# RainbowZL0/swin-unet-image-fusion

Hardware: AMD Instinct MI355X
Metric: fused image-pairs/sec at 256x256, win=8 (higher is better)
Workload: dtype bf16; 1 GPU; B=16/GPU 256x256 IR/visible pairs, win=8, 5-level Swin-UNet fusion forward (BASELINE configs[1]); global_batch=16, precision_mode=fast, residual_stream=fp32, hip_graph=True, steps_in_flight=3, kernel_schedule=throughput, collective=none, weights=random-init (numpy PCG64 recipe, seed 0)

## Files before the change

### swin_unet_image_fusion_amd/csrc/kernels_win24.hip

```cpp
#include "win_host.h"

namespace swf {
namespace {

using namespace wf;

constexpr int W24_WAVES = 3;

template <int HID_>
struct G24 {
    static constexpr int C = 24, HID = HID_, HEADS = 8, D = 3;
    static constexpr bool ONES_H = HID % 32 != 0;
    static constexpr int NT1 = (HID + (ONES_H ? 1 : 0) + 31) / 32;
    static constexpr int KU = (HID + (ONES_H ? 1 : 0) + 15) / 16;
    static constexpr int F_QKV = 0;
    static constexpr int F_P = 12;
    static constexpr int F_W1 = 16;
    static constexpr int F_W2 = F_W1 + 4 * NT1;
    static constexpr int NFRAG = F_W2 + 2 * KU;
    static constexpr size_t p_vec = size_t(NFRAG) * 1024;
    static constexpr int V_LN1G = 0, V_LN1B = 12, V_LN2G = 24, V_LN2B = 36, V_B2 = 48;
    static constexpr size_t p_bias = p_vec + 2 * 64 * 4;
    static constexpr size_t p_total = p_bias + size_t(2) * 2 * 16 * 64 * 4;
    static constexpr size_t l_k = 0, l_v = l_k + 16 * 1024, l_vec = l_v + 16 * 1024, l_total = l_vec + 2 * 2 * 64 * 4;
    static constexpr size_t p_total16 = p_bias + size_t(15) * 64 * 16 * 4;
    static constexpr size_t l_k16 = 0, l_v16 = 32 * 1024, l_vec16 = 64 * 1024, l_total16 = l_vec16 + 2 * 2 * 64 * 4;
};

__device__ __forceinline__ void layernorm_frags(const f32x16& res, const float* vec, int goff, int boff, u32x4 (&xh)[2], u32x4 (&xl)[2]) {
    float s = 0.f;
#pragma unroll
    for (int i = 0; i < 12; ++i) s += res[i];
    const float mean = sum_halves(s) * (1.0f / 24.0f);
    float d[12], q = 0.f;
#pragma unroll
    for (int i = 0; i < 12; ++i) {
        d[i] = res[i] - mean;
        q += d[i] * d[i];
    }
    const float rstd = __builtin_amdgcn_rsqf(sum_halves(q) * (1.0f / 24.0f) + 1e-5f);
    float n[16];
#pragma unroll
    for (int a = 0; a < 3; ++a) {
        const float4 g = *reinterpret_cast<const float4*>(vec + goff + 4 * a);
        const float4 b = *reinterpret_cast<const float4*>(vec + boff + 4 * a);
        n[4 * a + 0] = d[4 * a + 0] * rstd * g.x + b.x;
        n[4 * a + 1] = d[4 * a + 1] * rstd * g.y + b.y;
        n[4 * a + 2] = d[4 * a + 2] * rstd * g.z + b.z;
        n[4 * a + 3] = d[4 * a + 3] * rstd * g.w + b.w;
    }
    n[12] = 1.0f;
    n[13] = n[14] = n[15] = 0.f;
    split8(n, xh[0], xl[0]);
    split8(n + 8, xh[1], xl[1]);
}

__device__ __forceinline__ void raw_frags(const f32x16& res, u32x4 (&xh)[2], u32x4 (&xl)[2]) {
    float n[16];
#pragma unroll
    for (int i = 0; i < 12; ++i) n[i] = res[i];
    n[12] = 1.0f;
    n[13] = n[14] = n[15] = 0.f;
    split8(n, xh[0], xl[0]);
    split8(n + 8, xh[1], xl[1]);
}

template <bool ONLINE>
__device__ __forceinline__ f32x16 attention24(const u32x4* ksrc, const u32x4* vsrc, const u32x4 (&qf)[2], const f32x16 (&bias)[2], bool half1,
                                            f32x16 o, float* mrun = nullptr) {
    const f32x16 zero16 = {0.f, 0.f, 0.f, 0.f, 0.f, 0.f, 0.f, 0.f, 0.f, 0.f, 0.f, 0.f, 0.f, 0.f, 0.f, 0.f};
#pragma unroll
    for (int h = 0; h < 8; ++h) {
        const int s = h >> 2, sub = (h >> 1) & 1;
        const bool keep = half1 == ((h & 1) != 0);
        const u32x4 ka0 = ksrc[(0 * 2 + s) * 64], ka1 = ksrc[(1 * 2 + s) * 64];
        u32x4 qm = {0u, 0u, 0u, 0u};
        qm[2 * sub] = keep ? qf[s][2 * sub] : 0u;
        qm[2 * sub + 1] = keep ? qf[s][2 * sub + 1] : 0u;
        f32x16 s0 = mfma_f16(ka0, qm, bias[0]);
        f32x16 s1 = mfma_f16(ka1, qm, bias[1]);
        float mx = max3f(s0[0], s0[1], s1[0]);
        mx = max3f(mx, s1[1], s0[2]);
#pragma unroll
        for (int i = 3; i < 16; i += 2) mx = max3f(mx, s0[i], s0[i + 1 < 16 ? i + 1 : i]);
#pragma unroll
        for (int i = 2; i < 16; i += 2) mx = max3f(mx, s1[i], s1[i + 1]);
        mx = max_halves(mx);
        float alpha = 0.f;
        f16 nm = (f16)(-mx);
        if constexpr (ONLINE) {
            const float mold = mrun[h >> 1];
            nm = (f16)(-__builtin_fmaxf(mold, mx));
            const float mnew = -(float)nm;
            alpha = __builtin_amdgcn_exp2f(mold - mnew);
            mrun[h >> 1] = keep ? mnew : mold;
        }
        const unsigned nmb = keep ? (unsigned)__builtin_bit_cast(unsigned short, nm) : 0u;
        qm[2 * sub + 1] |= nmb << 16;
        s0 = mfma_f16(ka0, qm, bias[0]);
        s1 = mfma_f16(ka1, qm, bias[1]);
        f32x16 t;
#pragma unroll
        for (int ps = 0; ps < 4; ++ps) {
            float p[8];
#pragma unroll
            for (int j = 0; j < 8; ++j) p[j] = __builtin_amdgcn_exp2f((ps >> 1) ? s1[8 * (ps & 1) + j] : s0[8 * (ps & 1) + j]);
            const u32x4 pf = pack8_f16(p);
            const u32x4 va = vsrc[ps * 64];
            t = mfma_f16(va, pf, ps == 0 ? zero16 : t);
            __builtin_amdgcn_sched_barrier(0);
        }
#pragma unroll
        for (int j = 0; j < 4; ++j) {
            const int i = 4 * (h >> 1) + j;
            o[i] = keep ? (ONLINE ? __builtin_fmaf(o[i], alpha, t[i]) : t[i]) : o[i];
        }
        __builtin_amdgcn_sched_barrier(0);
    }
    return o;
}

__device__ __forceinline__ void load_rows24(const __amdgpu_buffer_rsrc_t& irs, unsigned tokoff, f32x16& dstv) {
#pragma unroll
    for (int a = 0; a < 3; ++a) {
        const f32x4 v = __builtin_bit_cast(f32x4, __builtin_amdgcn_raw_buffer_load_b128(irs, tokoff, 32 * a, 0));
        dstv[4 * a] = v.x; dstv[4 * a + 1] = v.y; dstv[4 * a + 2] = v.z; dstv[4 * a + 3] = v.w;
    }
    dstv[12] = dstv[13] = dstv[14] = dstv[15] = 0.f;
}
__device__ __forceinline__ void store_rows24(__amdgpu_buffer_rsrc_t ors, unsigned tokoff, f32x16 res) {
#pragma unroll
    for (int a = 0; a < 3; ++a) {
        const f32x4 v = {res[4 * a], res[4 * a + 1], res[4 * a + 2], res[4 * a + 3]};
        __builtin_amdgcn_raw_buffer_store_b128(__builtin_bit_cast(u32x4, v), ors, tokoff, 32 * a, 0);
    }
}

template <class G, class WFn>
__device__ __forceinline__ f32x16 project24(WFn WF, f32x16 o, f32x16 res) {
    float t[16];
#pragma unroll
    for (int a = 0; a < 4; ++a) {
        const float inv = __builtin_amdgcn_rcpf(o[4 * a + 3]);
        t[4 * a] = o[4 * a] * inv; t[4 * a + 1] = o[4 * a + 1] * inv; t[4 * a + 2] = o[4 * a + 2] * inv;
        t[4 * a + 3] = 1.0f;
    }
    u32x4 oh[2], ol[2];
    split8(t, oh[0], ol[0]);
// ... 16 lines not shown
    u32x4* kimg = reinterpret_cast<u32x4*>(smem + G::l_k);
    u32x4* vimg = reinterpret_cast<u32x4*>(smem + G::l_v);
    float* lvec = reinterpret_cast<float*>(smem + G::l_vec);

    const int tid = threadIdx.x, lane = tid & 63, wave = tid >> 6;
    const int ws = wave >> 1, qb = wave & 1, r = lane & 31, hf = lane >> 5;
    const int H = args.H, W = args.W, nwx = MLP && !ATT ? 1 : W / WS, nwy = MLP && !ATT ? 1 : H / WS, npi = nwx * nwy;
    const int nwin = ATT ? args.B * npi : (max(args.ntok[0], args.ntok[1]) + 63) / 64;
    const int sh = args.shift ? WS / 2 : 0;
    const int kvs = args.cross ? 1 - ws : ws;

    for (int i = tid; i < 2 * 2 * 64; i += 256) lvec[i] = reinterpret_cast<const float*>(args.packed[i >> 7] + G::p_vec)[i & 127];
    const __amdgpu_buffer_rsrc_t wrs = __builtin_amdgcn_make_buffer_rsrc(const_cast<char*>(uniform_ptr(args.packed[ws])), 0, (int)G::p_total, 0x00020000);
    const __amdgpu_buffer_rsrc_t krs = __builtin_amdgcn_make_buffer_rsrc(const_cast<char*>(uniform_ptr(args.packed[kvs])), 0, (int)G::p_total, 0x00020000);
    const int act_bytes = ATT ? args.B * H * W * 24 * 4 : args.ntok[ws] * 24 * 4;
    const __amdgpu_buffer_rsrc_t irs = __builtin_amdgcn_make_buffer_rsrc(const_cast<float*>(uniform_ptr(args.in[ws])), 0, act_bytes, 0x00020000);
    const __amdgpu_buffer_rsrc_t ors = __builtin_amdgcn_make_buffer_rsrc(uniform_ptr(args.out[ws]), 0, (MODE == WIN_BLOCK || args.out[ws]) ? act_bytes : 0, 0x00020000);
    const unsigned loff = (unsigned)lane * 16u;
    auto WF = [&](int f) { return __builtin_bit_cast(u32x4, __builtin_amdgcn_raw_buffer_load_b128(wrs, loff, f * 1024, 0)); };
    auto WK = [&](int f) { return __builtin_bit_cast(u32x4, __builtin_amdgcn_raw_buffer_load_b128(krs, loff, f * 1024, 0)); };
    const float* vec = lvec + (ws * 2 + hf) * 64;
    f32x16 bias[2];
    auto load_bias = [&]() {
        const int vo = lane * 128 + qb * (2 * 16 * 64 * 4);
#pragma unroll
        for (int kt = 0; kt < 2; ++kt)
#pragma unroll
            for (int q4 = 0; q4 < 4; ++q4) {
                const f32x4 t = __builtin_bit_cast(f32x4, __builtin_amdgcn_raw_buffer_load_b128(wrs, vo + (kt * 16 + q4 * 4) * 4, (int)G::p_bias, 0));
#pragma unroll
                for (int e = 0; e < 4; ++e) bias[kt][q4 * 4 + e] = t[e];
            }
    };
    if constexpr (ATT) load_bias();
    const bool half1 = hf != 0;
    const bool col_masked = half1 != (((r >> 2) & 1) != 0);
    __syncthreads();

    int it = 0;
    for (int win = blockIdx.x; win < nwin; win += gridDim.x, ++it) {
        SWF_WF_FENCE();
        const int b = win / npi, wrem = win - b * npi;
        const int wy = wrem / nwx, wx = wrem - wy * nwx;
        const int buf = it & 1;
        int lane_w = lane;
        asm volatile("" : "+v"(lane_w));
        const int ty = 4 * qb + ((lane_w >> 3) & 3), tx = lane_w & 7;
        unsigned oy = wy * WS + ty + sh, ox = wx * WS + tx + sh;
        oy = oy < oy - (unsigned)H ? oy : oy - (unsigned)H;
        ox = ox < ox - (unsigned)W ? ox : ox - (unsigned)W;
        const unsigned tokoff = [&]() -> unsigned {
            if constexpr (ATT) {
                return (WS == 8 || (ty < WS && tx < WS)) ? (unsigned)((((b * H + (int)oy) * W + (int)ox) * 24 + 4 * (lane_w >> 5)) * 4) : 0x80000000u;
            } else {
                const int tok = 64 * win + 32 * qb + (lane_w & 31);
                return tok < args.ntok[ws] ? (unsigned)((tok * 24 + 4 * (lane_w >> 5)) * 4) : 0x80000000u;
            }
        }();
        const f32x16 zero16 = {0.f, 0.f, 0.f, 0.f, 0.f, 0.f, 0.f, 0.f, 0.f, 0.f, 0.f, 0.f, 0.f, 0.f, 0.f, 0.f};

        f32x16 res;
        if constexpr (ATT) {
        u32x4 qf[2];
        {
            f32x16 x0;
            load_rows24(irs, tokoff, x0);
            u32x4 xh[2], xl[2];
            if constexpr (RAW) raw_frags(x0, xh, xl);
            else layernorm_frags(x0, vec, G::V_LN1G, G::V_LN1B, xh, xl);
            f32x16 acc = zero16;
            if (!(RAW && ws == 1)) {
#pragma unroll
                for (int s = 0; s < 2; ++s) acc = mma3(WF(G::F_QKV + 2 * s), WF(G::F_QKV + 2 * s + 1), xh[s], xl[s], acc);
                float t[16];
#pragma unroll
                for (int i = 0; i < 16; ++i) t[i] = acc[i];
                qf[0] = pack8_f16(t);
                qf[1] = pack8_f16(t + 8);
            }
            SWF_WF_FENCE();
            if (!(RAW && ws == 0)) {
                float t[16];
                acc = zero16;
#pragma unroll
                for (int s = 0; s < 2; ++s) acc = mma3(WK(G::F_QKV + 4 + 2 * s), WK(G::F_QKV + 5 + 2 * s), xh[s], xl[s], acc);
#pragma unroll
                for (int i = 0; i < 16; ++i) t[i] = acc[i];
                u32x4* kdst = kimg + (((buf * 2 + kvs) * 2 + qb) * 2) * 64 + lane;
                kdst[0] = pack8_f16(t);
                kdst[64] = pack8_f16(t + 8);
                SWF_WF_FENCE();
                acc = zero16;
#pragma unroll
                for (int s = 0; s < 2; ++s) acc = mma3(xh[s], xl[s], WK(G::F_QKV + 8 + 2 * s), WK(G::F_QKV + 9 + 2 * s), acc);
#pragma unroll
                for (int i = 0; i < 16; ++i) t[i] = acc[i];
                u32x4* vdst = vimg + ((buf * 2 + kvs) * 4 + 2 * qb) * 64 + lane;
                vdst[0] = pack8_f16(t);
                vdst[64] = pack8_f16(t + 8);
            }
        }
        __syncthreads();
        if (RAW && ws == 1) continue;

        f32x16 o;
        {
            const bool rowv = args.shift && wy == nwy - 1, colv = args.shift && wx == nwx - 1;
            const u32x4* ksrc = kimg + ((buf * 2 + ws) * 4) * 64 + lane;
            const u32x4* vsrc = vimg + ((buf * 2 + ws) * 4) * 64 + lane;
            if (rowv || colv) {
                const float pen0 = ((rowv && qb == 1) || (colv && col_masked)) ? -INFINITY : 0.f;
                const float pen1 = ((rowv && qb == 0) || (colv && col_masked)) ? -INFINITY : 0.f;
#pragma unroll
                for (int i = 0; i < 16; ++i) { bias[0][i] += pen0; bias[1][i] += pen1; }
            }
            o = attention24<false>(ksrc, vsrc, qf, bias, half1, zero16);
            if (rowv || colv) load_bias();
        }

        SWF_WF_FENCE();
        if constexpr (RAW) res = zero16;
        else load_rows24(irs, tokoff, res);
        res = project24<G>(WF, o, res);
        } else {
            load_rows24(irs, tokoff, res);
        }

        if constexpr (MLP) {
            u32x4 xh[2], xl[2];
            if constexpr (RAW) { raw_frags(res, xh, xl); res = zero16; }
            else layernorm_frags(res, vec, G::V_LN2G, G::V_LN2B, xh, xl);
#pragma unroll
            for (int tI = 0; tI < G::NT1; ++tI) {
                SWF_WF_FENCE();
                f32x16 acc = zero16;
#pragma unroll
                for (int s = 0; s < 2; ++s)
                    acc = mma3(WF(G::F_W1 + 4 * tI + 2 * s), WF(G::F_W1 + 4 * tI + 2 * s + 1), xh[s], xl[s], acc);
                float e[16];
                elu_tile(acc, e);
#pragma unroll
                for (int s2 = 0; s2 < 2; ++s2) {
                    const int u = 2 * tI + s2;
                    if (u < G::KU) {
                        u32x4 hh, hl;
                        split8(e + 8 * s2, hh, hl);
                        SWF_WF_FENCE();
                        res = mma3(WF(G::F_W2 + 2 * u), WF(G::F_W2 + 2 * u + 1), hh, hl, res);
                    }
                }
                __builtin_amdgcn_sched_barrier(0);
            }
            if constexpr (!G::ONES_H) {
#pragma unroll
                for (int a = 0; a < 3; ++a) {
// ... 6 lines not shown
        store_rows24(ors, tokoff, res);
    }

    if (args.warm[0]) warm_next_block<256>(args, tid);
}

template <int HID>
__global__ __launch_bounds__(256, 2) void window24w16_kernel(WinArgs args) {
    using G = G24<HID>;
    extern __shared__ __attribute__((aligned(16))) char smem16[];
    u32x4* kimg = reinterpret_cast<u32x4*>(smem16 + G::l_k16);
    u32x4* vimg = reinterpret_cast<u32x4*>(smem16 + G::l_v16);
    float* lvec = reinterpret_cast<float*>(smem16 + G::l_vec16);

    const int tid = threadIdx.x, lane = tid & 63, wave = tid >> 6;
    const int ws = wave >> 1, pw = wave & 1, r = lane & 31, hf = lane >> 5;
    const int H = args.H, W = args.W, nwx = W / 16, nwy = H / 16, npi = nwx * nwy;
    const int nwin = args.B * npi;
    const int sh = args.shift ? 8 : 0;
    const int kvs = args.cross ? 1 - ws : ws;

    for (int i = tid; i < 2 * 2 * 64; i += 256) lvec[i] = reinterpret_cast<const float*>(args.packed[i >> 7] + G::p_vec)[i & 127];
    const __amdgpu_buffer_rsrc_t wrs = __builtin_amdgcn_make_buffer_rsrc(const_cast<char*>(uniform_ptr(args.packed[ws])), 0, (int)G::p_total16, 0x00020000);
    const __amdgpu_buffer_rsrc_t krs = __builtin_amdgcn_make_buffer_rsrc(const_cast<char*>(uniform_ptr(args.packed[kvs])), 0, (int)G::p_total16, 0x00020000);
    const int act_bytes = args.B * H * W * 24 * 4;
    const __amdgpu_buffer_rsrc_t irs = __builtin_amdgcn_make_buffer_rsrc(const_cast<float*>(uniform_ptr(args.in[ws])), 0, act_bytes, 0x00020000);
    const __amdgpu_buffer_rsrc_t ors = __builtin_amdgcn_make_buffer_rsrc(uniform_ptr(args.out[ws]), 0, act_bytes, 0x00020000);
    const unsigned loff = (unsigned)lane * 16u;
    auto WF = [&](int f) { return __builtin_bit_cast(u32x4, __builtin_amdgcn_raw_buffer_load_b128(wrs, loff, f * 1024, 0)); };
    auto WK = [&](int f) { return __builtin_bit_cast(u32x4, __builtin_amdgcn_raw_buffer_load_b128(krs, loff, f * 1024, 0)); };
    const float* vec = lvec + (ws * 2 + hf) * 64;
    const bool half1 = hf != 0;
    const f32x16 zero16 = {0.f, 0.f, 0.f, 0.f, 0.f, 0.f, 0.f, 0.f, 0.f, 0.f, 0.f, 0.f, 0.f, 0.f, 0.f, 0.f};
    __syncthreads();

    for (int win = blockIdx.x; win < nwin; win += gridDim.x) {
        SWF_WF_FENCE();
        const int b = win / npi, wrem = win - b * npi;
        const int wy = wrem / nwx, wx = wrem - wy * nwx;
        auto tokoff_of = [&](int j) {
            int lane_w = lane;
            asm volatile("" : "+v"(lane_w));
            unsigned oy = wy * 16 + 2 * j + ((lane_w >> 4) & 1) + sh, ox = wx * 16 + (lane_w & 15) + sh;
            oy = oy < oy - (unsigned)H ? oy : oy - (unsigned)H;
            ox = ox < ox - (unsigned)W ? ox : ox - (unsigned)W;
            return (unsigned)((((b * H + (int)oy) * W + (int)ox) * 24 + 4 * (lane_w >> 5)) * 4);
        };

        u32x4 qf[4][2];
#pragma unroll
        for (int q = 0; q < 4; ++q) { qf[q][0] = u32x4{0u, 0u, 0u, 0u}; qf[q][1] = u32x4{0u, 0u, 0u, 0u}; }
        {
            u32x4 wq[4], wk[4], wv[4];
#pragma unroll
            for (int i = 0; i < 4; ++i) { wq[i] = WF(G::F_QKV + i); wk[i] = WK(G::F_QKV + 4 + i); wv[i] = WK(G::F_QKV + 8 + i); }
#pragma unroll 1
            for (int jj = 0; jj < 4; ++jj) {
                const int j = 4 * pw + jj;
                f32x16 x0;
                load_rows24(irs, tokoff_of(j), x0);
                u32x4 xh[2], xl[2];
                layernorm_frags(x0, vec, G::V_LN1G, G::V_LN1B, xh, xl);
                f32x16 acc = zero16;
#pragma unroll
                for (int s = 0; s < 2; ++s) acc = mma3(wq[2 * s], wq[2 * s + 1], xh[s], xl[s], acc);
                float t[16];
#pragma unroll
                for (int i = 0; i < 16; ++i) t[i] = acc[i];
#pragma unroll
                for (int q = 0; q < 3; ++q) { qf[q][0] = qf[q + 1][0]; qf[q][1] = qf[q + 1][1]; }
                qf[3][0] = pack8_f16(t);
                qf[3][1] = pack8_f16(t + 8);
                acc = zero16;
#pragma unroll
                for (int s = 0; s < 2; ++s) acc = mma3(wk[2 * s], wk[2 * s + 1], xh[s], xl[s], acc);
#pragma unroll
                for (int i = 0; i < 16; ++i) t[i] = acc[i];
                u32x4* kdst = kimg + ((kvs * 8 + j) * 2) * 64 + lane;
                kdst[0] = pack8_f16(t);
                kdst[64] = pack8_f16(t + 8);
                acc = zero16;
#pragma unroll
                for (int s = 0; s < 2; ++s) acc = mma3(xh[s], xl[s], wv[2 * s], wv[2 * s + 1], acc);
#pragma unroll
                for (int i = 0; i < 16; ++i) t[i] = acc[i];
                u32x4* vdst = vimg + (kvs * 16 + 2 * j) * 64 + lane;
                vdst[0] = pack8_f16(t);
                vdst[64] = pack8_f16(t + 8);
            }
        }
        __syncthreads();

        const bool rowv = args.shift && wy == nwy - 1, colv = args.shift && wx == nwx - 1;
        const u32x4* ksrc = kimg + (ws * 16) * 64 + lane;
        const u32x4* vsrc = vimg + (ws * 16) * 64 + lane;
#pragma unroll 1
        for (int jj = 0; jj < 4; ++jj) {
            const int j = 4 * pw + jj;
            const unsigned tokoff = tokoff_of(j);
            f32x16 o = zero16;
            float mrun[4] = {-INFINITY, -INFINITY, -INFINITY, -INFINITY};
#pragma unroll 1
            for (int c = 0; c < 4; ++c) {
                if (rowv && ((j < 4) != (c < 2))) continue;
                f32x16 bias[2];
                {
                    const int d0 = __builtin_amdgcn_readfirstlane(2 * c - j + 7);
#pragma unroll
                    for (int kt = 0; kt < 2; ++kt)
#pragma unroll
                        for (int q4 = 0; q4 < 4; ++q4) {
                            const f32x4 tb = __builtin_bit_cast(f32x4, __builtin_amdgcn_raw_buffer_load_b128(wrs, lane * 64 + q4 * 16, (int)G::p_bias + (d0 + kt) * 4096, 0));
#pragma unroll
                            for (int e = 0; e < 4; ++e) bias[kt][q4 * 4 + e] = tb[e];
                        }
                    if (colv) col_seam16(bias, r);
                }
                o = attention24<true>(ksrc + (2 * c) * 2 * 64, vsrc + (4 * c) * 64, qf[0], bias, half1, o, mrun);
            }
#pragma unroll
            for (int q = 0; q < 3; ++q) { qf[q][0] = qf[q + 1][0]; qf[q][1] = qf[q + 1][1]; }

            f32x16 res;
            SWF_WF_FENCE();
            load_rows24(irs, tokoff, res);
            res = project24<G>(WF, o, res);
            u32x4 xh[2], xl[2];
            layernorm_frags(res, vec, G::V_LN2G, G::V_LN2B, xh, xl);
#pragma unroll
            for (int tI = 0; tI < G::NT1; ++tI) {
                SWF_WF_FENCE();
                f32x16 acc = zero16;
#pragma unroll
                for (int s = 0; s < 2; ++s)
                    acc = mma3(WF(G::F_W1 + 4 * tI + 2 * s), WF(G::F_W1 + 4 * tI + 2 * s + 1), xh[s], xl[s], acc);
                float e[16];
                elu_tile(acc, e);
#pragma unroll
                for (int s2 = 0; s2 < 2; ++s2) {
                    const int u = 2 * tI + s2;
                    if (u < G::KU) {
                        u32x4 hh, hl;
                        split8(e + 8 * s2, hh, hl);
                        SWF_WF_FENCE();
                        res = mma3(WF(G::F_W2 + 2 * u), WF(G::F_W2 + 2 * u + 1), hh, hl, res);
                    }
                }
                __builtin_amdgcn_sched_barrier(0);
            }
            if constexpr (!G::ONES_H) {
#pragma unroll
// ... 102 lines not shown
```

### swin_unet_image_fusion_amd/csrc/kernels_win48.hip

```cpp
#include "win_host.h"

namespace swf {
namespace {

using namespace wf;

constexpr int W48_WAVES = 2;

template <int HID_>
struct G48 {
    static constexpr int C = 48, HID = HID_, HEADS = 8, D = 6;
    static constexpr int NT1 = HID / 32, KU = HID / 16;
    static_assert(HID % 32 == 0, "hidden tiles");
    static constexpr int F_QKV = 0;
    static constexpr int F_P = 36;
    static constexpr int F_W1 = 52;
    static constexpr int F_W2 = F_W1 + 6 * NT1;
    static constexpr int NFRAG = F_W2 + 4 * KU;
    static constexpr int V_LN1G = 0, V_LN1B = 24, V_LN2G = 48, V_LN2B = 72, V_B2 = 96, V_BQ = 120, V_BK = 152, V_B1 = 184, VHF = 288;
    static_assert(V_B1 + 16 * NT1 <= VHF, "vector block");
    static constexpr int VSTREAM = 2 * VHF + 64;
    static constexpr size_t p_vec = size_t(NFRAG) * 1024;
    static constexpr size_t p_bias = (p_vec + size_t(VSTREAM) * 4 + 15) / 16 * 16;
    static constexpr size_t p_total = p_bias + size_t(2) * 2 * 16 * 64 * 4;
    static constexpr size_t l_k = 0, l_v = 16 * 1024, l_vec = 32 * 1024, l_total = l_vec + size_t(2) * VSTREAM * 4;
    static constexpr size_t p_total16 = p_bias + size_t(15) * 16 * 64 * 4;
    static constexpr size_t l_k16 = 0, l_v16 = 32 * 1024, l_vec16 = 64 * 1024, l_total16 = l_vec16 + size_t(2) * VSTREAM * 4;
};


__device__ __forceinline__ void raw48(const f32x16& x0, const f32x16& x1, u32x4 (&xh)[3], u32x4 (&xl)[3]) {
    float n[24];
#pragma unroll
    for (int i = 0; i < 24; ++i) n[i] = i < 16 ? x0[i] : x1[i - 16];
    split8(n, xh[0], xl[0]);
    split8(n + 8, xh[1], xl[1]);
    split8(n + 16, xh[2], xl[2]);
}

__device__ __forceinline__ void layernorm48(const f32x16& x0, const f32x16& x1, const float* vec, int goff, int boff, u32x4 (&xh)[3], u32x4 (&xl)[3]) {
    float s = 0.f;
#pragma unroll
    for (int i = 0; i < 16; ++i) s += x0[i];
#pragma unroll
    for (int i = 0; i < 8; ++i) s += x1[i];
    const float mean = sum_halves(s) * (1.0f / 48.0f);
    float d[24], q = 0.f;
#pragma unroll
    for (int i = 0; i < 24; ++i) {
        d[i] = (i < 16 ? x0[i] : x1[i - 16]) - mean;
        q += d[i] * d[i];
    }
    const float rstd = __builtin_amdgcn_rsqf(sum_halves(q) * (1.0f / 48.0f) + 1e-5f);
    float n[24];
#pragma unroll
    for (int a = 0; a < 6; ++a) {
        const float4 g = *reinterpret_cast<const float4*>(vec + goff + 4 * a);
        const float4 b = *reinterpret_cast<const float4*>(vec + boff + 4 * a);
        n[4 * a + 0] = d[4 * a + 0] * rstd * g.x + b.x;
        n[4 * a + 1] = d[4 * a + 1] * rstd * g.y + b.y;
        n[4 * a + 2] = d[4 * a + 2] * rstd * g.z + b.z;
        n[4 * a + 3] = d[4 * a + 3] * rstd * g.w + b.w;
    }
    split8(n, xh[0], xl[0]);
    split8(n + 8, xh[1], xl[1]);
    split8(n + 16, xh[2], xl[2]);
}

template <bool ONLINE, int VSTEPS = 4>
__device__ __forceinline__ void attention48(const u32x4* ksrc, const u32x4* vsrc, const u32x4 (&qf)[2][2], const f32x16 (&bias)[2],
                                            bool half1, f32x16 (&o)[2], float* mrun = nullptr) {
    const f32x16 zero16 = {0.f, 0.f, 0.f, 0.f, 0.f, 0.f, 0.f, 0.f, 0.f, 0.f, 0.f, 0.f, 0.f, 0.f, 0.f, 0.f};
    if constexpr (!ONLINE) { o[0] = zero16; o[1] = zero16; }
#pragma unroll
    for (int h = 0; h < 8; ++h) {
        const int T = h >> 2, hq = h & 3, sp = hq >> 1, sub = hq & 1;
        const u32x4 ka0 = ksrc[((0 * 2 + T) * 2 + sp) * 64], ka1 = ksrc[((1 * 2 + T) * 2 + sp) * 64];
        u32x4 qm = {0u, 0u, 0u, 0u};
        qm[2 * sub] = qf[T][sp][2 * sub];
        qm[2 * sub + 1] = qf[T][sp][2 * sub + 1];
        float mx;
        {
            f32x16 s0 = mfma_f16(ka0, qm, bias[0]);
            mx = max3f(s0[0], s0[1], s0[2]);
#pragma unroll
            for (int i = 3; i < 15; i += 2) mx = max3f(mx, s0[i], s0[i + 1]);
            mx = __builtin_fmaxf(mx, s0[15]);
        }
        {
            f32x16 s1 = mfma_f16(ka1, qm, bias[1]);
#pragma unroll
            for (int i = 0; i < 16; i += 2) mx = max3f(mx, s1[i], s1[i + 1]);
        }
        mx = max_halves(mx);
        f16 nm = (f16)(-mx);
        float alpha = 0.f;
        if constexpr (ONLINE) {
            const float mold = mrun[h];
            nm = (f16)(-__builtin_fmaxf(mold, mx));
            const float mnew = -(float)nm;
            alpha = __builtin_amdgcn_exp2f(mold - mnew);
            mrun[h] = mnew;
        }
        qm[2 * sub + 1] |= half1 ? ((unsigned)__builtin_bit_cast(unsigned short, nm) << 16) : 0u;
        f32x16 t;
#pragma unroll
        for (int kt = 0; kt < 2; ++kt) {
            f32x16 sc = mfma_f16(kt ? ka1 : ka0, qm, bias[kt]);
#pragma unroll
            for (int s2 = 0; s2 < 2; ++s2) {
                float p[8];
#pragma unroll
                for (int j = 0; j < 8; ++j) p[j] = __builtin_amdgcn_exp2f(sc[8 * s2 + j]);
                const u32x4 pf = pack8_f16(p);
                const u32x4 va = vsrc[(T * VSTEPS + 2 * kt + s2) * 64];
                t = mfma_f16(va, pf, (kt == 0 && s2 == 0) ? zero16 : t);
                __builtin_amdgcn_sched_barrier(0);
            }
        }
#pragma unroll
        for (int j = 0; j < 4; ++j) o[T][4 * hq + j] = ONLINE ? __builtin_fmaf(o[T][4 * hq + j], alpha, t[4 * hq + j]) : t[4 * hq + j];
        __builtin_amdgcn_sched_barrier(0);
    }
}

template <int HID, int WS, int MODE = WIN_BLOCK, bool RAW = false>
__global__ __launch_bounds__(256, W48_WAVES) void window48_kernel(WinArgs args) {
    using G = G48<HID>;
    static_assert(WS == 7 || WS == 8, "window side");
    static_assert(!RAW || MODE != WIN_BLOCK, "RAW belongs to the half-block modes");
    constexpr bool ATT = MODE != WIN_MLP, MLP = MODE != WIN_ATTN;
    __shared__ __attribute__((aligned(16))) char smem[G::l_total];
    u32x4* kimg = reinterpret_cast<u32x4*>(smem + G::l_k);
    u32x4* vimg = reinterpret_cast<u32x4*>(smem + G::l_v);
    float* lvec = reinterpret_cast<float*>(smem + G::l_vec);

    const int tid = threadIdx.x, lane = tid & 63, wave = tid >> 6;
    const int ws = wave >> 1, qb = wave & 1, r = lane & 31, hf = lane >> 5;
    const int H = args.H, W = args.W, nwx = ATT ? W / WS : 1, nwy = ATT ? H / WS : 1, npi = nwx * nwy;
    const int nwin = ATT ? args.B * npi : (max(args.ntok[0], args.ntok[1]) + 63) / 64;
    const int sh = args.shift ? WS / 2 : 0;
    const int kvs = args.cross ? 1 - ws : ws;

    const __amdgpu_buffer_rsrc_t wrs = __builtin_amdgcn_make_buffer_rsrc(const_cast<char*>(uniform_ptr(args.packed[ws])), 0, (int)G::p_total, 0x00020000);
    const __amdgpu_buffer_rsrc_t krs = __builtin_amdgcn_make_buffer_rsrc(const_cast<char*>(uniform_ptr(args.packed[kvs])), 0, (int)G::p_total, 0x00020000);
    const int act_bytes = ATT ? args.B * H * W * 48 * 4 : args.ntok[ws] * 48 * 4;
    const __amdgpu_buffer_rsrc_t irs = __builtin_amdgcn_make_buffer_rsrc(const_cast<float*>(uniform_ptr(args.in[ws])), 0, act_bytes, 0x00020000);
    const __amdgpu_buffer_rsrc_t ors = __builtin_amdgcn_make_buffer_rsrc(uniform_ptr(args.out[ws]), 0, (MODE == WIN_BLOCK || args.out[ws]) ? act_bytes : 0, 0x00020000);
    const unsigned loff = (unsigned)lane * 16u;
    auto WF = [&](int f) { return __builtin_bit_cast(u32x4, __builtin_amdgcn_raw_buffer_load_b128(wrs, loff, f * 1024, 0)); };
    auto WK = [&](int f) { return __builtin_bit_cast(u32x4, __builtin_amdgcn_raw_buffer_load_b128(krs, loff, f * 1024, 0)); };
    const float* vec = lvec + ws * G::VSTREAM + hf * G::VHF;
    const float* veck = lvec + kvs * G::VSTREAM + hf * G::VHF;
    const float* vecv = lvec + kvs * G::VSTREAM + 2 * G::VHF;
    const bool half1 = hf != 0;
    const bool col_masked = half1 != (((r >> 2) & 1) != 0);
    const f32x16 zero16 = {0.f, 0.f, 0.f, 0.f, 0.f, 0.f, 0.f, 0.f, 0.f, 0.f, 0.f, 0.f, 0.f, 0.f, 0.f, 0.f};

    for (int win = blockIdx.x; win < nwin; win += gridDim.x) {
        SWF_WF_FENCE();
        const int b = win / npi, wrem = win - b * npi;
        const int wy = wrem / nwx, wx = wrem - wy * nwx;
        const int ty = 4 * qb + (r >> 3), tx = r & 7;
        int oy = wy * WS + ty + sh, ox = wx * WS + tx + sh;
        oy = oy >= H ? oy - H : oy;
        ox = ox >= W ? ox - W : ox;
        const unsigned tokoff = [&]() -> unsigned {
            if constexpr (ATT) {
                return (WS == 8 || (ty < WS && tx < WS)) ? (unsigned)((((b * H + oy) * W + ox) * 48 + 4 * hf) * 4) : 0x80000000u;
            } else {
                const int tok = 64 * win + 32 * qb + r;
                return tok < args.ntok[ws] ? (unsigned)((tok * 48 + 4 * hf) * 4) : 0x80000000u;
            }
        }();
        auto load_rows = [&](f32x16& t0, f32x16& t1) {
#pragma unroll
            for (int a = 0; a < 6; ++a) {
                const f32x4 v = __builtin_bit_cast(f32x4, __builtin_amdgcn_raw_buffer_load_b128(irs, tokoff, 32 * a, 0));
                if (a < 4) { t0[4 * a] = v.x; t0[4 * a + 1] = v.y; t0[4 * a + 2] = v.z; t0[4 * a + 3] = v.w; }
                else { t1[4 * (a - 4)] = v.x; t1[4 * (a - 4) + 1] = v.y; t1[4 * (a - 4) + 2] = v.z; t1[4 * (a - 4) + 3] = v.w; }
            }
#pragma unroll
            for (int i = 8; i < 16; ++i) t1[i] = 0.f;
        };

        f32x16 res0, res1;
        if constexpr (ATT) {
        u32x4 qf[2][2];
        {
            u32x4 wq[2][6];
            auto req = [&](int ph, u32x4 (&dst)[6]) {
                const int m = ph >> 1, T = ph & 1;
#pragma unroll
                for (int i = 0; i < 6; ++i) dst[i] = m == 0 ? WF(G::F_QKV + ((m * 2 + T) * 3) * 2 + i) : WK(G::F_QKV + ((m * 2 + T) * 3) * 2 + i);
            };
            req(0, wq[0]);
            f32x16 x0, x1;
            load_rows(x0, x1);
            if (win == (int)blockIdx.x) {
                static_assert(G::VSTREAM % 4 == 0 && G::p_vec % 16 == 0, "vector sections move as 16-byte groups");
                    fill_vectors<G::VSTREAM / 4, 256>(lvec, args.packed[0] + G::p_vec, args.packed[1] + G::p_vec, tid);
                __syncthreads();
            }
            u32x4 xh[3], xl[3];
            if constexpr (RAW) raw48(x0, x1, xh, xl);
            else layernorm48(x0, x1, vec, G::V_LN1G, G::V_LN1B, xh, xl);
            float t[16];
#pragma unroll
            for (int ph = 0; ph < 6; ++ph) {
                const int m = ph >> 1, T = ph & 1;
                SWF_WF_FENCE();
                if (ph + 1 < 6) req(ph + 1, wq[(ph + 1) & 1]);
                SWF_WF_FENCE();
                const u32x4 (&w)[6] = wq[ph & 1];
                f32x16 acc = zero16;
                if (RAW && (m == 0 ? ws == 1 : ws == 0)) {
                    if (ph == 2 && win != (int)blockIdx.x) __syncthreads();
                } else if (m < 2) {
#pragma unroll
                    for (int s = 0; s < 3; ++s) acc = mma3(w[2 * s], w[2 * s + 1], xh[s], xl[s], acc);
                    const float* bsrc = m == 0 ? vec + G::V_BQ : veck + G::V_BK;
#pragma unroll
                    for (int g = 0; g < 4; ++g) {
                        const float4 bb = *reinterpret_cast<const float4*>(bsrc + 16 * T + 4 * g);
                        t[4 * g] = acc[4 * g] + bb.x; t[4 * g + 1] = acc[4 * g + 1] + bb.y; t[4 * g + 2] = acc[4 * g + 2] + bb.z; t[4 * g + 3] = acc[4 * g + 3] + bb.w;
                    }
                    if (m == 0) {
                        qf[T][0] = pack8_f16(t);
                        qf[T][1] = pack8_f16(t + 8);
                    } else {
                        if (T == 0 && win != (int)blockIdx.x) __syncthreads();
                        u32x4* kdst = kimg + (((kvs * 2 + qb) * 2 + T) * 2) * 64 + lane;
                        kdst[0] = pack8_f16(t);
                        kdst[64] = pack8_f16(t + 8);
                    }
                } else {
#pragma unroll
                    for (int s = 0; s < 3; ++s) acc = mma3(xh[s], xl[s], w[2 * s], w[2 * s + 1], acc);
                    const float bv = vecv[32 * T + r];
#pragma unroll
                    for (int i = 0; i < 16; ++i) t[i] = acc[i] + bv;
                    u32x4* vdst = vimg + ((kvs * 2 + T) * 4 + 2 * qb) * 64 + lane;
                    vdst[0] = pack8_f16(t);
                    vdst[64] = pack8_f16(t + 8);
                }
            }
        }
        f32x16 bias[2];
        load_bias_tiles(wrs, loff, (int)G::p_bias, __builtin_amdgcn_readfirstlane(qb) * 2, bias);
        __syncthreads();
        if (RAW && ws == 1) continue;

        f32x16 o[2];
        {
            const bool rowv = args.shift && wy == nwy - 1, colv = args.shift && wx == nwx - 1;
            const u32x4* ksrc = kimg + (ws * 8) * 64 + lane;
            const u32x4* vsrc = vimg + (ws * 8) * 64 + lane;
            if (rowv || colv) {
                const float pen0 = ((rowv && qb == 1) || (colv && col_masked)) ? -INFINITY : 0.f;
                const float pen1 = ((rowv && qb == 0) || (colv && col_masked)) ? -INFINITY : 0.f;
#pragma unroll
                for (int i = 0; i < 16; ++i) { bias[0][i] += pen0; bias[1][i] += pen1; }
            }
            attention48<false>(ksrc, vsrc, qf, bias, half1, o);
        }

        u32x4 wpj[16];
        SWF_WF_FENCE();
        if constexpr (RAW) { res0 = zero16; res1 = zero16; }
        else load_rows(res0, res1);
#pragma unroll
        for (int i = 0; i < 16; ++i) wpj[i] = WF(G::F_P + i);
        SWF_WF_FENCE();
        {
            u32x4 oh[4], ol[4];
#pragma unroll
            for (int T = 0; T < 2; ++T) {
                float t[16];
#pragma unroll
                for (int q = 0; q < 4; ++q) {
                    float lo_, den;
                    halves(o[T][4 * q + 2], lo_, den);
                    const float inv = __builtin_amdgcn_rcpf(den);
                    t[4 * q] = o[T][4 * q] * inv; t[4 * q + 1] = o[T][4 * q + 1] * inv; t[4 * q + 2] = o[T][4 * q + 2] * inv; t[4 * q + 3] = o[T][4 * q + 3] * inv;
                }
                split8(t, oh[2 * T], ol[2 * T]);
                split8(t + 8, oh[2 * T + 1], ol[2 * T + 1]);
            }
#pragma unroll
            for (int ks = 0; ks < 4; ++ks) {
                res0 = mma3(wpj[(0 * 4 + ks) * 2], wpj[(0 * 4 + ks) * 2 + 1], oh[ks], ol[ks], res0);
                res1 = mma3(wpj[(1 * 4 + ks) * 2], wpj[(1 * 4 + ks) * 2 + 1], oh[ks], ol[ks], res1);
            }
        }

        } else {
            load_rows(res0, res1);
            if (win == (int)blockIdx.x) {
                fill_vectors<G::VSTREAM / 4, 256>(lvec, args.packed[0] + G::p_vec, args.packed[1] + G::p_vec, tid);
                __syncthreads();
            }
        }

// ... 56 lines not shown

    if (args.warm[0]) warm_next_block<256>(args, tid);
}

template <int HID>
__global__ __launch_bounds__(256, 2) void window48w16_kernel(WinArgs args) {
    using G = G48<HID>;
    extern __shared__ __attribute__((aligned(16))) char smem48[];
    u32x4* kimg = reinterpret_cast<u32x4*>(smem48 + G::l_k16);
    u32x4* vimg = reinterpret_cast<u32x4*>(smem48 + G::l_v16);
    float* lvec = reinterpret_cast<float*>(smem48 + G::l_vec16);

    const int tid = threadIdx.x, lane = tid & 63, wave = tid >> 6;
    const int ws = blockIdx.y, r = lane & 31, hf = lane >> 5;
    const int H = args.H, W = args.W, nwx = W / 16, nwy = H / 16, npi = nwx * nwy;
    const int nwin = args.B * npi;
    const int sh = args.shift ? 8 : 0;
    const int src = args.cross ? 1 - ws : ws;

    static_assert(G::VSTREAM % 4 == 0 && G::p_vec % 16 == 0, "vector sections move as 16-byte groups");
                    fill_vectors<G::VSTREAM / 4, 256>(lvec, args.packed[0] + G::p_vec, args.packed[1] + G::p_vec, tid);
    const __amdgpu_buffer_rsrc_t wrs = __builtin_amdgcn_make_buffer_rsrc(const_cast<char*>(args.packed[ws]), 0, (int)G::p_total16, 0x00020000);
    const int act_bytes = args.B * H * W * 48 * 4;
    const __amdgpu_buffer_rsrc_t irs = __builtin_amdgcn_make_buffer_rsrc(const_cast<float*>(args.in[ws]), 0, act_bytes, 0x00020000);
    const __amdgpu_buffer_rsrc_t srs = __builtin_amdgcn_make_buffer_rsrc(const_cast<float*>(args.in[src]), 0, act_bytes, 0x00020000);
    const __amdgpu_buffer_rsrc_t ors = __builtin_amdgcn_make_buffer_rsrc(args.out[ws], 0, act_bytes, 0x00020000);
    const unsigned loff = (unsigned)lane * 16u;
    auto WF = [&](int f) { return __builtin_bit_cast(u32x4, __builtin_amdgcn_raw_buffer_load_b128(wrs, loff, f * 1024, 0)); };
    const float* vec = lvec + ws * G::VSTREAM + hf * G::VHF;
    const float* vecs = lvec + src * G::VSTREAM + hf * G::VHF;
    const float* vecv = lvec + ws * G::VSTREAM + 2 * G::VHF;
    const bool half1 = hf != 0;
    const f32x16 zero16 = {0.f, 0.f, 0.f, 0.f, 0.f, 0.f, 0.f, 0.f, 0.f, 0.f, 0.f, 0.f, 0.f, 0.f, 0.f, 0.f};
    __syncthreads();

    for (int win = blockIdx.x; win < nwin; win += gridDim.x) {
        SWF_WF_FENCE();
        const int b = win / npi, wrem = win - b * npi;
        const int wy = wrem / nwx, wx = wrem - wy * nwx;
        auto tokoff_of = [&](int j) {
            int oy = wy * 16 + 2 * j + (r >> 4) + sh, ox = wx * 16 + (r & 15) + sh;
            oy = oy >= H ? oy - H : oy;
            ox = ox >= W ? ox - W : ox;
            return (unsigned)((((b * H + oy) * W + ox) * 48 + 4 * hf) * 4);
        };
        auto load_rows = [&](const __amdgpu_buffer_rsrc_t& rs, unsigned tokoff, f32x16& t0, f32x16& t1) {
#pragma unroll
            for (int a = 0; a < 6; ++a) {
                const f32x4 v = __builtin_bit_cast(f32x4, __builtin_amdgcn_raw_buffer_load_b128(rs, tokoff, 32 * a, 0));
                if (a < 4) { t0[4 * a] = v.x; t0[4 * a + 1] = v.y; t0[4 * a + 2] = v.z; t0[4 * a + 3] = v.w; }
                else { t1[4 * (a - 4)] = v.x; t1[4 * (a - 4) + 1] = v.y; t1[4 * (a - 4) + 2] = v.z; t1[4 * (a - 4) + 3] = v.w; }
            }
#pragma unroll
            for (int i = 8; i < 16; ++i) t1[i] = 0.f;
        };

        u32x4 qf[2][2][2];
        {
            u32x4 xh[2][3], xl[2][3], kh[2][3], kl[2][3];
#pragma unroll
            for (int jj = 0; jj < 2; ++jj) {
                const unsigned tokoff = tokoff_of(2 * wave + jj);
                f32x16 x0, x1;
                load_rows(irs, tokoff, x0, x1);
                layernorm48(x0, x1, vec, G::V_LN1G, G::V_LN1B, xh[jj], xl[jj]);
                if (args.cross) {
// ... 43 lines not shown
                    } else {
#pragma unroll
                        for (int s2 = 0; s2 < 3; ++s2) acc = mma3(kh[jj][s2], kl[jj][s2], w[2 * s2], w[2 * s2 + 1], acc);
                        const float bv = vecv[32 * T + r];
#pragma unroll
                        for (int i = 0; i < 16; ++i) t[i] = acc[i] + bv;
                        u32x4* vdst = vimg + (T * 16 + 2 * j) * 64 + lane;
                        vdst[0] = pack8_f16(t);
                        vdst[64] = pack8_f16(t + 8);
                    }
                }
            }
        }
        __syncthreads();

        const bool rowv = args.shift && wy == nwy - 1, colv = args.shift && wx == nwx - 1;
#pragma unroll 1
        for (int jj = 0; jj < 2; ++jj) {
            const int j = 2 * wave + jj;
            const unsigned tokoff = tokoff_of(j);
            f32x16 o[2] = {zero16, zero16};
            float mrun[8];
#pragma unroll
            for (int h = 0; h < 8; ++h) mrun[h] = -INFINITY;
#pragma unroll 1
            for (int c = 0; c < 4; ++c) {
                if (rowv && ((j < 4) != (c < 2))) continue;
                f32x16 bias[2];
                {
                    const int d0 = __builtin_amdgcn_readfirstlane(2 * c - j + 7);
                    load_bias_tiles(wrs, loff, (int)G::p_bias, d0, bias);
                    if (colv) col_seam16(bias, r);
                }
                attention48<true, 16>(kimg + (2 * c) * 4 * 64 + lane, vimg + (4 * c) * 64 + lane, qf[0], bias, half1, o, mrun);
            }
#pragma unroll
            for (int T = 0; T < 2; ++T) { qf[0][T][0] = qf[1][T][0]; qf[0][T][1] = qf[1][T][1]; }

            f32x16 res0, res1;
            SWF_WF_FENCE();
            load_rows(irs, tokoff, res0, res1);
            {
                u32x4 oh[4], ol[4];
#pragma unroll
                for (int T = 0; T < 2; ++T) {
                    float t[16];
#pragma unroll
                    for (int q = 0; q < 4; ++q) {
                        float lo_, den;
                        halves(o[T][4 * q + 2], lo_, den);
                        const float inv = __builtin_amdgcn_rcpf(den);
                        t[4 * q] = o[T][4 * q] * inv; t[4 * q + 1] = o[T][4 * q + 1] * inv; t[4 * q + 2] = o[T][4 * q + 2] * inv; t[4 * q + 3] = o[T][4 * q + 3] * inv;
                    }
                    split8(t, oh[2 * T], ol[2 * T]);
                    split8(t + 8, oh[2 * T + 1], ol[2 * T + 1]);
                }
                SWF_WF_FENCE();
#pragma unroll
                for (int ks = 0; ks < 4; ++ks) {
                    res0 = mma3(WF(G::F_P + (0 * 4 + ks) * 2), WF(G::F_P + (0 * 4 + ks) * 2 + 1), oh[ks], ol[ks], res0);
                    res1 = mma3(WF(G::F_P + (1 * 4 + ks) * 2), WF(G::F_P + (1 * 4 + ks) * 2 + 1), oh[ks], ol[ks], res1);
                }
            }
            {
                u32x4 w1[2][6];
                auto req1 = [&](int tI, u32x4 (&dst)[6]) {
#pragma unroll
// ... 149 lines not shown
```

### swin_unet_image_fusion_amd/csrc/win_frag.h

```cpp
#pragma once
#include <hip/hip_runtime.h>

namespace swf {
namespace wf {

using bf16 = __bf16;
using f16 = _Float16;
typedef bf16 bf16x8 __attribute__((ext_vector_type(8)));
typedef bf16 bf16x4 __attribute__((ext_vector_type(4)));
typedef bf16 bf16x2 __attribute__((ext_vector_type(2)));
typedef f16 f16x8 __attribute__((ext_vector_type(8)));
typedef f16 f16x4 __attribute__((ext_vector_type(4)));
typedef f16 f16x2 __attribute__((ext_vector_type(2)));
typedef float f32x16 __attribute__((ext_vector_type(16)));
typedef float f32x4 __attribute__((ext_vector_type(4)));
typedef unsigned u32x4 __attribute__((ext_vector_type(4)));

constexpr float kLog2e = 1.4426950408889634f, kLn2 = 0.6931471805599453f;

__host__ __device__ constexpr int rho(int i, int hf) { return (i & 3) + 8 * (i >> 2) + 4 * hf; }

__device__ __forceinline__ f32x16 mfma_bf16(u32x4 a, u32x4 b, f32x16 c) {
    return __builtin_amdgcn_mfma_f32_32x32x16_bf16(__builtin_bit_cast(bf16x8, a), __builtin_bit_cast(bf16x8, b), c, 0, 0, 0);
}
__device__ __forceinline__ f32x16 mfma_f16(u32x4 a, u32x4 b, f32x16 c) {
    return __builtin_amdgcn_mfma_f32_32x32x16_f16(__builtin_bit_cast(f16x8, a), __builtin_bit_cast(f16x8, b), c, 0, 0, 0);
}
__device__ __forceinline__ f32x16 mma3(u32x4 ahi, u32x4 alo, u32x4 bhi, u32x4 blo, f32x16 acc) {
    acc = mfma_bf16(alo, bhi, acc);
    acc = mfma_bf16(ahi, blo, acc);
    acc = mfma_bf16(ahi, bhi, acc);
    return acc;
}
__device__ __forceinline__ void split8(const float* v, u32x4& hi, u32x4& lo) {
#pragma unroll
    for (int p = 0; p < 4; ++p) {
        const bf16x2 h = {(bf16)v[2 * p], (bf16)v[2 * p + 1]};
        const unsigned hu = __builtin_bit_cast(unsigned, h);
        const float h0 = __builtin_bit_cast(float, hu << 16), h1 = __builtin_bit_cast(float, hu & 0xffff0000u);
        const bf16x2 l = {(bf16)(v[2 * p] - h0), (bf16)(v[2 * p + 1] - h1)};
        hi[p] = hu;
        lo[p] = __builtin_bit_cast(unsigned, l);
    }
}
__device__ __forceinline__ void split4(const float4 v, bf16x4& hi, bf16x4& lo) {
    const float f[4] = {v.x, v.y, v.z, v.w};
#pragma unroll
    for (int i = 0; i < 4; ++i) {
        hi[i] = (bf16)f[i];
        lo[i] = (bf16)(f[i] - (float)hi[i]);
    }
}
__device__ __forceinline__ u32x4 pack8_f16(const float* v) {
    u32x4 o;
#pragma unroll
    for (int p = 0; p < 4; ++p) {
        const f16x2 h = {(f16)v[2 * p], (f16)v[2 * p + 1]};
        o[p] = __builtin_bit_cast(unsigned, h);
    }
    return o;
// ... 98 lines not shown
```

Before: 9334 pairs/s.

## Use 16x16x32 MFMA for attention PV product with zero-padded V lanes

Replaces the 32x32x16 MFMA in the P·V step of the win24 and win48 attention kernels with the smaller 16x16x32 MFMA, which produces only the 4 output values each lane keeps. Lanes whose fragment does not match read from a new zero-filled LDS region instead, so each head computes only what it needs. The residual row load is also reused from the earlier load for layernorm instead of being reloaded before projection. The cost is extra LDS per block for the zero region and per-lane address selection, and the new fragment mapping must be correct.

```diff
diff --git a/swin_unet_image_fusion_amd/csrc/kernels_win24.hip b/swin_unet_image_fusion_amd/csrc/kernels_win24.hip
--- a/swin_unet_image_fusion_amd/csrc/kernels_win24.hip
+++ b/swin_unet_image_fusion_amd/csrc/kernels_win24.hip
@@ -22,9 +22,10 @@
     static constexpr int V_LN1G = 0, V_LN1B = 12, V_LN2G = 24, V_LN2B = 36, V_B2 = 48;
     static constexpr size_t p_bias = p_vec + 2 * 64 * 4;
     static constexpr size_t p_total = p_bias + size_t(2) * 2 * 16 * 64 * 4;
-    static constexpr size_t l_k = 0, l_v = l_k + 16 * 1024, l_vec = l_v + 16 * 1024, l_total = l_vec + 2 * 2 * 64 * 4;
+    static constexpr size_t l_k = 0, l_v = l_k + 16 * 1024, l_vec = l_v + 16 * 1024, l_zero = l_vec + 2 * 2 * 64 * 4,
+                            l_total = l_zero + kPvZeroBytes;
     static constexpr size_t p_total16 = p_bias + size_t(15) * 64 * 16 * 4;
-    static constexpr size_t l_k16 = 0, l_v16 = 32 * 1024, l_vec16 = 64 * 1024, l_total16 = l_vec16 + 2 * 2 * 64 * 4;
+    static constexpr size_t l_k16 = 0, l_v16 = 32 * 1024, l_vec16 = 64 * 1024, l_zero16 = l_vec16 + 2 * 2 * 64 * 4, l_total16 = l_zero16 + kPvZeroBytes;
 };
 
 __device__ __forceinline__ void layernorm_frags(const f32x16& res, const float* vec, int goff, int boff, u32x4 (&xh)[2], u32x4 (&xl)[2]) {
@@ -65,10 +66,14 @@
     split8(n + 8, xh[1], xl[1]);
 }
 
+__device__ __forceinline__ const u32x4* pv_src24(const char* smem, int lane, unsigned vblk, unsigned zreg) {
+    const unsigned off = pv_match(lane) ? vblk + (unsigned)(((lane & 32) + (lane & 3)) * 16) : zreg + (unsigned)kPvZeroBase;
+    return reinterpret_cast<const u32x4*>(smem + off);
+}
+
 template <bool ONLINE>
 __device__ __forceinline__ f32x16 attention24(const u32x4* ksrc, const u32x4* vsrc, const u32x4 (&qf)[2], const f32x16 (&bias)[2], bool half1,
                                             f32x16 o, float* mrun = nullptr) {
-    const f32x16 zero16 = {0.f, 0.f, 0.f, 0.f, 0.f, 0.f, 0.f, 0.f, 0.f, 0.f, 0.f, 0.f, 0.f, 0.f, 0.f, 0.f};
 #pragma unroll
     for (int h = 0; h < 8; ++h) {
         const int s = h >> 2, sub = (h >> 1) & 1;
@@ -99,21 +104,21 @@
         qm[2 * sub + 1] |= nmb << 16;
         s0 = mfma_f16(ka0, qm, bias[0]);
         s1 = mfma_f16(ka1, qm, bias[1]);
-        f32x16 t;
+        f32x4 t;
 #pragma unroll
         for (int ps = 0; ps < 4; ++ps) {
             float p[8];
 #pragma unroll
             for (int j = 0; j < 8; ++j) p[j] = __builtin_amdgcn_exp2f((ps >> 1) ? s1[8 * (ps & 1) + j] : s0[8 * (ps & 1) + j]);
             const u32x4 pf = pack8_f16(p);
-            const u32x4 va = vsrc[ps * 64];
-            t = mfma_f16(va, pf, ps == 0 ? zero16 : t);
+            const u32x4 va = vsrc[ps * 64 + h * 4];
+            t = mfma16_f16(va, pf, ps == 0 ? f32x4{0.f, 0.f, 0.f, 0.f} : t);
             __builtin_amdgcn_sched_barrier(0);
         }
 #pragma unroll
         for (int j = 0; j < 4; ++j) {
             const int i = 4 * (h >> 1) + j;
-            o[i] = keep ? (ONLINE ? __builtin_fmaf(o[i], alpha, t[i]) : t[i]) : o[i];
+            o[i] = keep ? (ONLINE ? __builtin_fmaf(o[i], alpha, t[j]) : t[j]) : o[i];
         }
         __builtin_amdgcn_sched_barrier(0);
     }
@@ -196,7 +201,10 @@
                 for (int e = 0; e < 4; ++e) bias[kt][q4 * 4 + e] = t[e];
             }
     };
-    if constexpr (ATT) load_bias();
+    if constexpr (ATT) {
+        load_bias();
+        pv_fill_zeros<256>(smem + G::l_zero, tid);
+    }
     const bool half1 = hf != 0;
     const bool col_masked = half1 != (((r >> 2) & 1) != 0);
     __syncthreads();
@@ -227,11 +235,10 @@
         if constexpr (ATT) {
         u32x4 qf[2];
         {
-            f32x16 x0;
-            load_rows24(irs, tokoff, x0);
+            load_rows24(irs, tokoff, res);
             u32x4 xh[2], xl[2];
-            if constexpr (RAW) raw_frags(x0, xh, xl);
-            else layernorm_frags(x0, vec, G::V_LN1G, G::V_LN1B, xh, xl);
+            if constexpr (RAW) raw_frags(res, xh, xl);
+            else layernorm_frags(res, vec, G::V_LN1G, G::V_LN1B, xh, xl);
             f32x16 acc = zero16;
             if (!(RAW && ws == 1)) {
 #pragma unroll
@@ -271,7 +278,7 @@
         {
             const bool rowv = args.shift && wy == nwy - 1, colv = args.shift && wx == nwx - 1;
             const u32x4* ksrc = kimg + ((buf * 2 + ws) * 4) * 64 + lane;
-            const u32x4* vsrc = vimg + ((buf * 2 + ws) * 4) * 64 + lane;
+            const u32x4* vsrc = pv_src24(smem, lane_w, (unsigned)(G::l_v + ((buf * 2 + ws) * 4) * 1024), (unsigned)G::l_zero);
             if (rowv || colv) {
                 const float pen0 = ((rowv && qb == 1) || (colv && col_masked)) ? -INFINITY : 0.f;
                 const float pen1 = ((rowv && qb == 0) || (colv && col_masked)) ? -INFINITY : 0.f;
@@ -284,7 +291,6 @@
 
         SWF_WF_FENCE();
         if constexpr (RAW) res = zero16;
-        else load_rows24(irs, tokoff, res);
         res = project24<G>(WF, o, res);
         } else {
             load_rows24(irs, tokoff, res);
@@ -357,6 +363,7 @@
     const float* vec = lvec + (ws * 2 + hf) * 64;
     const bool half1 = hf != 0;
     const f32x16 zero16 = {0.f, 0.f, 0.f, 0.f, 0.f, 0.f, 0.f, 0.f, 0.f, 0.f, 0.f, 0.f, 0.f, 0.f, 0.f, 0.f};
+    pv_fill_zeros<256>(smem16 + G::l_zero16, tid);
     __syncthreads();
 
     for (int win = blockIdx.x; win < nwin; win += gridDim.x) {
@@ -418,7 +425,6 @@
 
         const bool rowv = args.shift && wy == nwy - 1, colv = args.shift && wx == nwx - 1;
         const u32x4* ksrc = kimg + (ws * 16) * 64 + lane;
-        const u32x4* vsrc = vimg + (ws * 16) * 64 + lane;
 #pragma unroll 1
         for (int jj = 0; jj < 4; ++jj) {
             const int j = 4 * pw + jj;
@@ -441,7 +447,8 @@
                         }
                     if (colv) col_seam16(bias, r);
                 }
-                o = attention24<true>(ksrc + (2 * c) * 2 * 64, vsrc + (4 * c) * 64, qf[0], bias, half1, o, mrun);
+                const u32x4* vsrc = pv_src24(smem16, lane, (unsigned)(G::l_v16 + (ws * 16 + 4 * c) * 1024), (unsigned)G::l_zero16);
+                o = attention24<true>(ksrc + (2 * c) * 2 * 64, vsrc, qf[0], bias, half1, o, mrun);
             }
 #pragma unroll
             for (int q = 0; q < 3; ++q) { qf[q][0] = qf[q + 1][0]; qf[q][1] = qf[q + 1][1]; }
diff --git a/swin_unet_image_fusion_amd/csrc/kernels_win48.hip b/swin_unet_image_fusion_amd/csrc/kernels_win48.hip
--- a/swin_unet_image_fusion_amd/csrc/kernels_win48.hip
+++ b/swin_unet_image_fusion_amd/csrc/kernels_win48.hip
@@ -23,9 +23,9 @@
     static constexpr size_t p_vec = size_t(NFRAG) * 1024;
     static constexpr size_t p_bias = (p_vec + size_t(VSTREAM) * 4 + 15) / 16 * 16;
     static constexpr size_t p_total = p_bias + size_t(2) * 2 * 16 * 64 * 4;
-    static constexpr size_t l_k = 0, l_v = 16 * 1024, l_vec = 32 * 1024, l_total = l_vec + size_t(2) * VSTREAM * 4;
+    static constexpr size_t l_k = 0, l_v = 16 * 1024, l_vec = 32 * 1024, l_zero = l_vec + size_t(2) * VSTREAM * 4, l_total = l_zero + kPvZeroBytes;
     static constexpr size_t p_total16 = p_bias + size_t(15) * 16 * 64 * 4;
-    static constexpr size_t l_k16 = 0, l_v16 = 32 * 1024, l_vec16 = 64 * 1024, l_total16 = l_vec16 + size_t(2) * VSTREAM * 4;
+    static constexpr size_t l_k16 = 0, l_v16 = 32 * 1024, l_vec16 = 64 * 1024, l_zero16 = l_vec16 + size_t(2) * VSTREAM * 4, l_total16 = l_zero16 + kPvZeroBytes;
 };
 
 
@@ -67,8 +67,13 @@
     split8(n + 16, xh[2], xl[2]);
 }
 
-template <bool ONLINE, int VSTEPS = 4>
-__device__ __forceinline__ void attention48(const u32x4* ksrc, const u32x4* vsrc, const u32x4 (&qf)[2][2], const f32x16 (&bias)[2],
+__device__ __forceinline__ const u32x4* pv_src48(const char* smem, int lane, unsigned vblk, unsigned zreg) {
+    const unsigned off = pv_match(lane) ? vblk + (unsigned)(((lane & 32) + ((lane >> 1) & 4) + (lane & 3)) * 16) : zreg + (unsigned)kPvZeroBase;
+    return reinterpret_cast<const u32x4*>(smem + off);
+}
+
+template <bool ONLINE>
+__device__ __forceinline__ void attention48(const u32x4* ksrc, const u32x4* const (&vsrc)[2], const u32x4 (&qf)[2][2], const f32x16 (&bias)[2],
                                             bool half1, f32x16 (&o)[2], float* mrun = nullptr) {
     const f32x16 zero16 = {0.f, 0.f, 0.f, 0.f, 0.f, 0.f, 0.f, 0.f, 0.f, 0.f, 0.f, 0.f, 0.f, 0.f, 0.f, 0.f};
     if constexpr (!ONLINE) { o[0] = zero16; o[1] = zero16; }
@@ -103,7 +108,7 @@
             mrun[h] = mnew;
         }
         qm[2 * sub + 1] |= half1 ? ((unsigned)__builtin_bit_cast(unsigned short, nm) << 16) : 0u;
-        f32x16 t;
+        f32x4 t;
 #pragma unroll
         for (int kt = 0; kt < 2; ++kt) {
             f32x16 sc = mfma_f16(kt ? ka1 : ka0, qm, bias[kt]);
@@ -113,13 +118,13 @@
 #pragma unroll
                 for (int j = 0; j < 8; ++j) p[j] = __builtin_amdgcn_exp2f(sc[8 * s2 + j]);
                 const u32x4 pf = pack8_f16(p);
-                const u32x4 va = vsrc[(T * VSTEPS + 2 * kt + s2) * 64];
-                t = mfma_f16(va, pf, (kt == 0 && s2 == 0) ? zero16 : t);
+                const u32x4 va = vsrc[T][(2 * kt + s2) * 64 + hq * 8];
+                t = mfma16_f16(va, pf, (kt == 0 && s2 == 0) ? f32x4{0.f, 0.f, 0.f, 0.f} : t);
                 __builtin_amdgcn_sched_barrier(0);
             }
         }
 #pragma unroll
-        for (int j = 0; j < 4; ++j) o[T][4 * hq + j] = ONLINE ? __builtin_fmaf(o[T][4 * hq + j], alpha, t[4 * hq + j]) : t[4 * hq + j];
+        for (int j = 0; j < 4; ++j) o[T][4 * hq + j] = ONLINE ? __builtin_fmaf(o[T][4 * hq + j], alpha, t[j]) : t[j];
         __builtin_amdgcn_sched_barrier(0);
     }
 }
@@ -156,6 +161,7 @@
     const bool half1 = hf != 0;
     const bool col_masked = half1 != (((r >> 2) & 1) != 0);
     const f32x16 zero16 = {0.f, 0.f, 0.f, 0.f, 0.f, 0.f, 0.f, 0.f, 0.f, 0.f, 0.f, 0.f, 0.f, 0.f, 0.f, 0.f};
+    if constexpr (ATT) pv_fill_zeros<256>(smem + G::l_zero, tid);
 
     for (int win = blockIdx.x; win < nwin; win += gridDim.x) {
         SWF_WF_FENCE();
@@ -195,7 +201,7 @@
                 for (int i = 0; i < 6; ++i) dst[i] = m == 0 ? WF(G::F_QKV + ((m * 2 + T) * 3) * 2 + i) : WK(G::F_QKV + ((m * 2 + T) * 3) * 2 + i);
             };
             req(0, wq[0]);
-            f32x16 x0, x1;
+            f32x16 &x0 = res0, &x1 = res1;
             load_rows(x0, x1);
             if (win == (int)blockIdx.x) {
                 static_assert(G::VSTREAM % 4 == 0 && G::p_vec % 16 == 0, "vector sections move as 16-byte groups");
@@ -255,7 +261,8 @@
         {
             const bool rowv = args.shift && wy == nwy - 1, colv = args.shift && wx == nwx - 1;
             const u32x4* ksrc = kimg + (ws * 8) * 64 + lane;
-            const u32x4* vsrc = vimg + (ws * 8) * 64 + lane;
+            const u32x4* const vsrc[2] = {pv_src48(smem, lane, (unsigned)(G::l_v + (ws * 8) * 1024), (unsigned)G::l_zero),
+                                          pv_src48(smem, lane, (unsigned)(G::l_v + (ws * 8 + 4) * 1024), (unsigned)G::l_zero)};
             if (rowv || colv) {
                 const float pen0 = ((rowv && qb == 1) || (colv && col_masked)) ? -INFINITY : 0.f;
                 const float pen1 = ((rowv && qb == 0) || (colv && col_masked)) ? -INFINITY : 0.f;
@@ -268,7 +275,6 @@
         u32x4 wpj[16];
         SWF_WF_FENCE();
         if constexpr (RAW) { res0 = zero16; res1 = zero16; }
-        else load_rows(res0, res1);
 #pragma unroll
         for (int i = 0; i < 16; ++i) wpj[i] = WF(G::F_P + i);
         SWF_WF_FENCE();
@@ -391,6 +397,7 @@
     const float* vecv = lvec + ws * G::VSTREAM + 2 * G::VHF;
     const bool half1 = hf != 0;
     const f32x16 zero16 = {0.f, 0.f, 0.f, 0.f, 0.f, 0.f, 0.f, 0.f, 0.f, 0.f, 0.f, 0.f, 0.f, 0.f, 0.f, 0.f};
+    pv_fill_zeros<256>(smem48 + G::l_zero16, tid);
     __syncthreads();
 
     for (int win = blockIdx.x; win < nwin; win += gridDim.x) {
@@ -500,7 +507,9 @@
                     load_bias_tiles(wrs, loff, (int)G::p_bias, d0, bias);
                     if (colv) col_seam16(bias, r);
                 }
-                attention48<true, 16>(kimg + (2 * c) * 4 * 64 + lane, vimg + (4 * c) * 64 + lane, qf[0], bias, half1, o, mrun);
+                const u32x4* const vsrc[2] = {pv_src48(smem48, lane, (unsigned)(G::l_v16 + (4 * c) * 1024), (unsigned)G::l_zero16),
+                                              pv_src48(smem48, lane, (unsigned)(G::l_v16 + (16 + 4 * c) * 1024), (unsigned)G::l_zero16)};
+                attention48<true>(kimg + (2 * c) * 4 * 64 + lane, vsrc, qf[0], bias, half1, o, mrun);
             }
 #pragma unroll
             for (int T = 0; T < 2; ++T) { qf[0][T][0] = qf[1][T][0]; qf[0][T][1] = qf[1][T][1]; }
diff --git a/swin_unet_image_fusion_amd/csrc/win_frag.h b/swin_unet_image_fusion_amd/csrc/win_frag.h
--- a/swin_unet_image_fusion_amd/csrc/win_frag.h
+++ b/swin_unet_image_fusion_amd/csrc/win_frag.h
@@ -26,6 +26,17 @@
 __device__ __forceinline__ f32x16 mfma_f16(u32x4 a, u32x4 b, f32x16 c) {
     return __builtin_amdgcn_mfma_f32_32x32x16_f16(__builtin_bit_cast(f16x8, a), __builtin_bit_cast(f16x8, b), c, 0, 0, 0);
 }
+__device__ __forceinline__ f32x4 mfma16_f16(u32x4 a, u32x4 b, f32x4 c) {
+    return __builtin_amdgcn_mfma_f32_16x16x32_f16(__builtin_bit_cast(f16x8, a), __builtin_bit_cast(f16x8, b), c, 0, 0, 0);
+}
+__device__ __forceinline__ bool pv_match(int lane) { return ((lane >> 4) & 1) == ((lane >> 2) & 1); }
+constexpr int kPvZeroBytes = 4096, kPvZeroBase = 128;
+static_assert(kPvZeroBase + 3 * 1024 + 7 * 64 + 16 <= kPvZeroBytes, "zero region covers every immediate");
+template <int NTHREADS>
+__device__ __forceinline__ void pv_fill_zeros(char* zreg, int tid) {
+    for (int i = tid; i < kPvZeroBytes / 16; i += NTHREADS) reinterpret_cast<u32x4*>(zreg)[i] = u32x4{0u, 0u, 0u, 0u};
+}
+
 __device__ __forceinline__ f32x16 mma3(u32x4 ahi, u32x4 alo, u32x4 bhi, u32x4 blo, f32x16 acc) {
     acc = mfma_bf16(alo, bhi, acc);
     acc = mfma_bf16(ahi, blo, acc);
```

Result: faster. 9688 pairs/s, median of 6 (+3.8%).
